# rogermm14/eonerf_code

Hardware: AMD Instinct MI355X
Metric: train rays/sec on JAX_068 (4096 rays x 128 samples) (higher is better)
Workload: dtype bf16

## Files before the change

eonerf_code_amd/csrc/eonerf_enc_pair.hip:

```cpp
#include "eonerf_common.h"
#include "eonerf_kernels.h"

namespace {

constexpr int NT = 512;
constexpr int IMG = 16 * 1024;
constexpr int ENC_B = ENC_SLOTS * SEG_B;
constexpr int SLOT_B = 2 * IMG + ENC_B;
constexpr int NS = 4, DEPTH = NS - 1;
constexpr int N_DMA = 9;
constexpr int GP_F = 4 * 32 * 4;
constexpr int SMEM_B = NS * SLOT_B + 2 * GP_F * (int)sizeof(float);

EO_DEV int swz16(int row, int chunk) { return (chunk ^ ((row >> 2) & 3)) * 16; }

EO_DEV void enc_waves(const EncPairArgs& a, uint8_t* smem, int lane, int wave, int t0, int t1, int n_pts) {
    typedef PBf16 P;
    typedef P::U U;
    const int h = lane >> 5, c = lane & 31;
    const int s_src = wave >> 1, mt = wave & 1;
    U wt[16];
#pragma unroll
    for (int kg = 0; kg < 16; ++kg) wt[kg] = *reinterpret_cast<const U*>(a.wt + ((size_t)((s_src * 2 + mt) * 16 + kg)) * 1024 + lane * 16);
    float* gp_lds = reinterpret_cast<float*>(smem + NS * SLOT_B);
    const float eoff = h ? EO_PI_2_F : 0.0f;
    auto load_pos = [&](int t, float& x, float& y, float& z) {
        const int p = t * 32 + c;
        const bool live = p < n_pts;
        x = live ? a.px[p] : 0.f; y = live ? a.py[p] : 0.f; z = live ? a.pz[p] : 0.f;
    };
    auto finish = [&](int t_prev, int par) {
        const int p = t_prev * 32 + c;
        if (h == 0 && p < n_pts) {
            const f32x4* g = reinterpret_cast<const f32x4*>(gp_lds + par * GP_F);
            f32x4 v = g[c];
#pragma unroll
            for (int w = 1; w < 4; ++w) { const f32x4 u = g[w * 32 + c]; v[0] += u[0]; v[1] += u[1]; v[2] += u[2]; }
            a.g_pos[p] = v[0]; a.g_pos[(size_t)a.p_pad + p] = v[1]; a.g_pos[2 * (size_t)a.p_pad + p] = v[2];
        }
    };
    float x, y, z;
    load_pos(t0, x, y, z);
    for (int t = t0; t < t1; ++t) {
        const int slot = (t - t0) & (NS - 1), par = (t - t0) & 1;
        asm volatile("s_barrier" ::: "memory");
        if (wave == 0 && t > t0) finish(t - 1, par ^ 1);
        const uint8_t* bp = smem + slot * SLOT_B + s_src * IMG + lane * 16;
        f32x16 acc = zero_acc();
        U fr[3];
#pragma unroll
        for (int d = 0; d < 3; ++d) fr[d] = lds_unit<P>(bp + d * 1024);
#pragma unroll
        for (int kg = 0; kg < 16; ++kg) {
            acc = P::mma(wt[kg], fr[kg % 3], acc);
            if (kg + 3 < 16) fr[kg % 3] = lds_unit<P>(bp + (kg + 3) * 1024);
        }
        float gp[3] = {0.f, 0.f, 0.f};
#pragma unroll
        for (int r = 0; r < 16; ++r) {
            const float g = acc[r];
            if (mt == 0 || r < 14) {
                const int q0 = r, q1 = 16 + r;
                const int k = mt ? q1 / 3 : q0 / 3, d = mt ? q1 % 3 : q0 % 3;
                const float cc = d == 0 ? x : (d == 1 ? y : z);
                const float arg = cc * (float)(1 << k) + eoff;
                gp[d] += g * (__cosf(arg) * (float)(1 << k));
            } else if (r == 14) {
                if (h) gp[2] += g; else gp[0] += g;
            } else {
                if (!h) gp[1] += g;
            }
        }
#pragma unroll
        for (int d = 0; d < 3; ++d) gp[d] += __shfl_xor(gp[d], 32, 64);
        if (h == 0) reinterpret_cast<f32x4*>(gp_lds + par * GP_F)[wave * 32 + c] = f32x4{gp[0], gp[1], gp[2], 0.f};
        if (t + 1 < t1) load_pos(t + 1, x, y, z);
    }
    asm volatile("s_barrier" ::: "memory");
    if (wave == 0) finish(t1 - 1, (t1 - 1 - t0) & 1);
}

EO_DEV void dw_waves(const EncPairArgs& a, uint8_t* smem, int lane, int wave, int t0, int t1) {
    typedef PBf16 P;
    typedef P::U U;
    const int h = lane >> 5, c = lane & 31, v = wave - 4;
    const int s_src = v >> 1, mhalf = v & 1;
    const size_t nt = (size_t)a.p_pad / 32;
    const uint8_t* grd = reinterpret_cast<const uint8_t*>(a.grd);
    const __amdgpu_buffer_rsrc_t rs_y0 = __builtin_amdgcn_make_buffer_rsrc(const_cast<uint8_t*>(grd) + (size_t)GRD_ROW_Y0 * nt * SEG_B, 0, -1, 0x00020000);
    const __amdgpu_buffer_rsrc_t rs_y5 = __builtin_amdgcn_make_buffer_rsrc(const_cast<uint8_t*>(grd) + (size_t)(GRD_ROW_Y0 + 5 * 256) * nt * SEG_B, 0, -1, 0x00020000);
    const __amdgpu_buffer_rsrc_t rs_e = __builtin_amdgcn_make_buffer_rsrc(const_cast<uint8_t*>(reinterpret_cast<const uint8_t*>(a.act)) + (size_t)ACT_ROW_ENC * nt * SEG_B, 0, -1, 0x00020000);
    const int enc_row = 16 * v + (lane >> 2);
    const int enc_voff = enc_row * SEG_B + (((lane & 3) ^ ((enc_row >> 2) & 3)) * 16);
    auto issue = [&](int t, int slot) {
        uint8_t* base = smem + slot * SLOT_B;
        const uint32_t so = (uint32_t)t * IMG;
#pragma unroll
        for (int i = 0; i < 4; ++i) {
            __builtin_amdgcn_raw_ptr_buffer_load_lds(rs_y0, (__attribute__((address_space(3))) void*)(base + (4 * v + i) * 1024), 16, lane * 16 + (4 * v + i) * 1024, so, 0, 2);
            __builtin_amdgcn_raw_ptr_buffer_load_lds(rs_y5, (__attribute__((address_space(3))) void*)(base + IMG + (4 * v + i) * 1024), 16, lane * 16 + (4 * v + i) * 1024, so, 0, 2);
        }
        __builtin_amdgcn_raw_ptr_buffer_load_lds(rs_e, (__attribute__((address_space(3))) void*)(base + 2 * IMG + 16 * v * SEG_B), 16, enc_voff, (uint32_t)t * ENC_B, 0, 2);
    };
    f32x16 dw[4][2];
    float dbv[4] = {0.f, 0.f, 0.f, 0.f};
#pragma unroll
    for (int i = 0; i < 4; ++i) { dw[i][0] = zero_acc(); dw[i][1] = zero_acc(); }
    const int g4 = lane >> 4, qq = (lane & 15) >> 2, pp = lane & 3;
    int off_a[4];
#pragma unroll
    for (int i = 0; i < 4; ++i)
        off_a[i] = s_src * IMG + (2 * (4 * mhalf + i) + (g4 & 1)) * 1024 + ((pp & 1) * 32 + 8 * (g4 >> 1) + qq) * 16 + (pp >> 1) * 8;
    int off_b[2][2];
#pragma unroll
    for (int j = 0; j < 2; ++j)
#pragma unroll
        for (int ks = 0; ks < 2; ++ks) { const int row = 32 * j + c; off_b[j][ks] = 2 * IMG + row * SEG_B + swz16(row, 2 * ks + h); }

#pragma unroll
    for (int d = 0; d < DEPTH; ++d) issue(t0 + d < t1 ? t0 + d : t1 - 1, d);
    for (int t = t0; t < t1; ++t) {
        const int slot = (t - t0) & (NS - 1);
        asm volatile("s_waitcnt vmcnt(%0)\n\ts_barrier" ::"n"(N_DMA * (DEPTH - 1)) : "memory");
        issue(t + DEPTH < t1 ? t + DEPTH : t1 - 1, (slot + DEPTH) & (NS - 1));
        const uint8_t* T = smem + slot * SLOT_B;
#pragma unroll
        for (int ks = 0; ks < 2; ++ks) {
            u32x2 ta[8];
            asm volatile("ds_read_b64_tr_b16 %0, %8\n\t"
                         "ds_read_b64_tr_b16 %1, %8 offset:64\n\t"
                         "ds_read_b64_tr_b16 %2, %9\n\t"
                         "ds_read_b64_tr_b16 %3, %9 offset:64\n\t"
                         "ds_read_b64_tr_b16 %4, %10\n\t"
                         "ds_read_b64_tr_b16 %5, %10 offset:64\n\t"
                         "ds_read_b64_tr_b16 %6, %11\n\t"
                         "ds_read_b64_tr_b16 %7, %11 offset:64\n\t"
                         "s_waitcnt lgkmcnt(0)"
                         : "=&v"(ta[0]), "=&v"(ta[1]), "=&v"(ta[2]), "=&v"(ta[3]), "=&v"(ta[4]), "=&v"(ta[5]), "=&v"(ta[6]), "=&v"(ta[7])
                         : "v"((uint32_t)(uintptr_t)(T + off_a[0] + 256 * ks)), "v"((uint32_t)(uintptr_t)(T + off_a[1] + 256 * ks)),
                           "v"((uint32_t)(uintptr_t)(T + off_a[2] + 256 * ks)), "v"((uint32_t)(uintptr_t)(T + off_a[3] + 256 * ks)) : "memory");
            const U b0 = lds_unit<P>(T + off_b[0][ks]), b1 = lds_unit<P>(T + off_b[1][ks]);
#pragma unroll
            for (int i = 0; i < 4; ++i) {
                const u32x4 av = u32x4{ta[2 * i][0], ta[2 * i][1], ta[2 * i + 1][0], ta[2 * i + 1][1]};
                const U af = __builtin_bit_cast(U, av);
                dw[i][0] = P::mma(af, b0, dw[i][0]);
                dw[i][1] = P::mma(af, b1, dw[i][1]);
                if (s_src == 0) {
#pragma unroll
                    for (int e = 0; e < 4; ++e) dbv[i] += __uint_as_float(av[e] << 16) + __uint_as_float(av[e] & 0xffff0000u);
                }
            }
        }
    }
    asm volatile("s_waitcnt vmcnt(0)" ::: "memory");
    float* part = a.part + (size_t)blockIdx.x * ENC_PART_F + (size_t)s_src * 256 * 64;
#pragma unroll
    for (int i = 0; i < 4; ++i)
#pragma unroll
        for (int j = 0; j < 2; ++j)
#pragma unroll
            for (int g = 0; g < 16; ++g) part[((4 * mhalf + i) * 32 + acc_row(g, h)) * 64 + 32 * j + c] = dw[i][j][g];
    if (s_src == 0) {
#pragma unroll
        for (int i = 0; i < 4; ++i) {
            const float sum = dbv[i] + __shfl_xor(dbv[i], 32, 64);
            if (h == 0) a.part[(size_t)blockIdx.x * ENC_PART_F + 2 * 256 * 64 + (4 * mhalf + i) * 32 + c] = sum;
        }
    }
}

__global__ __launch_bounds__(NT) void k_enc_pair(EncPairArgs a) {
    extern __shared__ __attribute__((aligned(16))) uint8_t smem[];
    const int lane = threadIdx.x & 63, wave = __builtin_amdgcn_readfirstlane(threadIdx.x >> 6);
    const int n_pts = *a.n_pts;
    const int n_tiles = (n_pts + 255) / 256 * 8;
    const int t0 = (int)((long long)blockIdx.x * n_tiles / gridDim.x), t1 = (int)((long long)(blockIdx.x + 1) * n_tiles / gridDim.x);
    if (t0 >= t1) {
        for (int i = threadIdx.x; i < ENC_PART_F; i += NT) a.part[(size_t)blockIdx.x * ENC_PART_F + i] = 0.f;
        return;
    }
    if (wave < 4) enc_waves(a, smem, lane, wave, t0, t1, n_pts);
    else dw_waves(a, smem, lane, wave, t0, t1);
}

}

hipError_t eo_launch_enc_pair(const EncPairArgs& a, int n_wg, hipStream_t st) {
    static EoAttrOnce attr;
    {
        const hipError_t e = attr.ensure([&] { return hipFuncSetAttribute(reinterpret_cast<const void*>(&k_enc_pair), hipFuncAttributeMaxDynamicSharedMemorySize, SMEM_B); });
        if (e != hipSuccess) return e;
    }
    hipLaunchKernelGGL(k_enc_pair, dim3(n_wg), dim3(NT), SMEM_B, st, a);
    return hipGetLastError();
}
```

Baseline: 1.244 million.

## Interleave encoding cosines with MMAs and spread DMA issue across dw compute

The encoder waves are templated on the M-tile so the cosine/frequency factors are compile-time indexed and computed between MFMA steps, with sched barriers enforcing the interleave. Position loads become buffer loads with bounds-checked descriptors and are prefetched two tiles ahead. The final gradient write is now spread across all four waves using masked buffer stores. In the dW waves, the per-tile DMA issue is split into pieces placed between MFMAs, LDS reads for both k-steps are issued up front, and fine-grained lgkmcnt waits replace the full drain. The aim is to hide the cosine latency and the LDS/DMA latency behind matrix work, at the cost of more registers and more fragile hand-written wait counts.

Result: no change. 1.250 million, median of 6 (+0.5%).

```diff
diff --git a/eonerf_code_amd/csrc/eonerf_enc_pair.hip b/eonerf_code_amd/csrc/eonerf_enc_pair.hip
--- a/eonerf_code_amd/csrc/eonerf_enc_pair.hip
+++ b/eonerf_code_amd/csrc/eonerf_enc_pair.hip
@@ -14,57 +14,75 @@
 
 EO_DEV int swz16(int row, int chunk) { return (chunk ^ ((row >> 2) & 3)) * 16; }
 
-EO_DEV void enc_waves(const EncPairArgs& a, uint8_t* smem, int lane, int wave, int t0, int t1, int n_pts) {
+template <int MT> EO_DEV void enc_waves(const EncPairArgs& a, uint8_t* smem, int lane, int wave, int t0, int t1, int n_pts) {
     typedef PBf16 P;
     typedef P::U U;
     const int h = lane >> 5, c = lane & 31;
-    const int s_src = wave >> 1, mt = wave & 1;
+    const int s_src = wave >> 1;
     U wt[16];
 #pragma unroll
-    for (int kg = 0; kg < 16; ++kg) wt[kg] = *reinterpret_cast<const U*>(a.wt + ((size_t)((s_src * 2 + mt) * 16 + kg)) * 1024 + lane * 16);
+    for (int kg = 0; kg < 16; ++kg) wt[kg] = *reinterpret_cast<const U*>(a.wt + ((size_t)((s_src * 2 + MT) * 16 + kg)) * 1024 + lane * 16);
     float* gp_lds = reinterpret_cast<float*>(smem + NS * SLOT_B);
     const float eoff = h ? EO_PI_2_F : 0.0f;
+    const uint32_t pos_b = (uint32_t)n_pts * 4u;
+    const __amdgpu_buffer_rsrc_t rs_x = __builtin_amdgcn_make_buffer_rsrc(const_cast<float*>(a.px), 0, pos_b, 0x00020000);
+    const __amdgpu_buffer_rsrc_t rs_y = __builtin_amdgcn_make_buffer_rsrc(const_cast<float*>(a.py), 0, pos_b, 0x00020000);
+    const __amdgpu_buffer_rsrc_t rs_z = __builtin_amdgcn_make_buffer_rsrc(const_cast<float*>(a.pz), 0, pos_b, 0x00020000);
+    const __amdgpu_buffer_rsrc_t rs_g = __builtin_amdgcn_make_buffer_rsrc(a.g_pos, 0, 3u * (uint32_t)a.p_pad * 4u, 0x00020000);
+    constexpr uint32_t DROP = 0x80000000u;
     auto load_pos = [&](int t, float& x, float& y, float& z) {
-        const int p = t * 32 + c;
-        const bool live = p < n_pts;
-        x = live ? a.px[p] : 0.f; y = live ? a.py[p] : 0.f; z = live ? a.pz[p] : 0.f;
-    };
-    auto finish = [&](int t_prev, int par) {
+        const uint32_t vo = (uint32_t)(t * 32 + c) * 4u;
+        x = __uint_as_float(__builtin_amdgcn_raw_buffer_load_b32(rs_x, vo, 0, 0));
+        y = __uint_as_float(__builtin_amdgcn_raw_buffer_load_b32(rs_y, vo, 0, 0));
+        z = __uint_as_float(__builtin_amdgcn_raw_buffer_load_b32(rs_z, vo, 0, 0));
+    };
+    auto finish = [&](int t_prev, int par, bool on) {
         const int p = t_prev * 32 + c;
-        if (h == 0 && p < n_pts) {
-            const f32x4* g = reinterpret_cast<const f32x4*>(gp_lds + par * GP_F);
-            f32x4 v = g[c];
-#pragma unroll
-            for (int w = 1; w < 4; ++w) { const f32x4 u = g[w * 32 + c]; v[0] += u[0]; v[1] += u[1]; v[2] += u[2]; }
-            a.g_pos[p] = v[0]; a.g_pos[(size_t)a.p_pad + p] = v[1]; a.g_pos[2 * (size_t)a.p_pad + p] = v[2];
-        }
-    };
-    float x, y, z;
-    load_pos(t0, x, y, z);
-    for (int t = t0; t < t1; ++t) {
-        const int slot = (t - t0) & (NS - 1), par = (t - t0) & 1;
+        const f32x4* g = reinterpret_cast<const f32x4*>(gp_lds + par * GP_F);
+        f32x4 v = g[c];
+#pragma unroll
+        for (int w = 1; w < 4; ++w) { const f32x4 u = g[w * 32 + c]; v[0] += u[0]; v[1] += u[1]; v[2] += u[2]; }
+        const bool mine = on && h == 0 && (c >> 3) == wave && p < n_pts;
+        const uint32_t vo = mine ? (uint32_t)p * 4u : DROP;
+        const uint32_t row = (uint32_t)a.p_pad * 4u;
+        __builtin_amdgcn_raw_buffer_store_b32(__float_as_uint(v[0]), rs_g, vo, 0, 0);
+        __builtin_amdgcn_raw_buffer_store_b32(__float_as_uint(v[1]), rs_g, vo, row, 0);
+        __builtin_amdgcn_raw_buffer_store_b32(__float_as_uint(v[2]), rs_g, vo, 2 * row, 0);
+    };
+#pragma unroll
+    for (int kg = 0; kg < 16; ++kg) asm volatile("" ::"v"(wt[kg]));
+    auto step = [&](int t, int par, float& x, float& y, float& z) {
+        const int slot = (t - t0) & (NS - 1);
         asm volatile("s_barrier" ::: "memory");
-        if (wave == 0 && t > t0) finish(t - 1, par ^ 1);
         const uint8_t* bp = smem + slot * SLOT_B + s_src * IMG + lane * 16;
         f32x16 acc = zero_acc();
+        float cf[16];
         U fr[3];
 #pragma unroll
         for (int d = 0; d < 3; ++d) fr[d] = lds_unit<P>(bp + d * 1024);
+        __builtin_amdgcn_sched_barrier(0);
 #pragma unroll
         for (int kg = 0; kg < 16; ++kg) {
             acc = P::mma(wt[kg], fr[kg % 3], acc);
             if (kg + 3 < 16) fr[kg % 3] = lds_unit<P>(bp + (kg + 3) * 1024);
-        }
+            constexpr int Q0 = 16 * MT;
+            if (Q0 + kg < 30) {
+                const int k = (Q0 + kg) / 3, d = (Q0 + kg) % 3;
+                const float cc = d == 0 ? x : (d == 1 ? y : z);
+                const float arg = __builtin_fmaf(cc, (float)(1 << k), eoff);
+                cf[kg] = __cosf(arg) * (float)(1 << k);
+            } else {
+                cf[kg] = 0.f;
+            }
+            __builtin_amdgcn_sched_barrier(0);
+        }
+        finish(t - 1, par ^ 1, t > t0);
         float gp[3] = {0.f, 0.f, 0.f};
 #pragma unroll
         for (int r = 0; r < 16; ++r) {
             const float g = acc[r];
-            if (mt == 0 || r < 14) {
-                const int q0 = r, q1 = 16 + r;
-                const int k = mt ? q1 / 3 : q0 / 3, d = mt ? q1 % 3 : q0 % 3;
-                const float cc = d == 0 ? x : (d == 1 ? y : z);
-                const float arg = cc * (float)(1 << k) + eoff;
-                gp[d] += g * (__cosf(arg) * (float)(1 << k));
+            if (MT == 0 || r < 14) {
+                gp[(16 * MT + r) % 3] = __builtin_fmaf(g, cf[r], gp[(16 * MT + r) % 3]);
             } else if (r == 14) {
                 if (h) gp[2] += g; else gp[0] += g;
             } else {
@@ -74,10 +92,19 @@
 #pragma unroll
         for (int d = 0; d < 3; ++d) gp[d] += __shfl_xor(gp[d], 32, 64);
         if (h == 0) reinterpret_cast<f32x4*>(gp_lds + par * GP_F)[wave * 32 + c] = f32x4{gp[0], gp[1], gp[2], 0.f};
-        if (t + 1 < t1) load_pos(t + 1, x, y, z);
+        load_pos(t + 2 < t1 ? t + 2 : t1 - 1, x, y, z);
+    };
+    float xa, ya, za, xb, yb, zb;
+    load_pos(t0, xa, ya, za);
+    finish(t0, 0, false);
+    load_pos(t0 + 1 < t1 ? t0 + 1 : t0, xb, yb, zb);
+    for (int t = t0; t < t1; t += 2) {
+        step(t, 0, xa, ya, za);
+        if (t + 1 >= t1) break;
+        step(t + 1, 1, xb, yb, zb);
     }
     asm volatile("s_barrier" ::: "memory");
-    if (wave == 0) finish(t1 - 1, (t1 - 1 - t0) & 1);
+    finish(t1 - 1, (t1 - 1 - t0) & 1, true);
 }
 
 EO_DEV void dw_waves(const EncPairArgs& a, uint8_t* smem, int lane, int wave, int t0, int t1) {
@@ -92,15 +119,13 @@
     const __amdgpu_buffer_rsrc_t rs_e = __builtin_amdgcn_make_buffer_rsrc(const_cast<uint8_t*>(reinterpret_cast<const uint8_t*>(a.act)) + (size_t)ACT_ROW_ENC * nt * SEG_B, 0, -1, 0x00020000);
     const int enc_row = 16 * v + (lane >> 2);
     const int enc_voff = enc_row * SEG_B + (((lane & 3) ^ ((enc_row >> 2) & 3)) * 16);
-    auto issue = [&](int t, int slot) {
+    auto issue_piece = [&](int t, int slot, int n) {
         uint8_t* base = smem + slot * SLOT_B;
         const uint32_t so = (uint32_t)t * IMG;
-#pragma unroll
-        for (int i = 0; i < 4; ++i) {
-            __builtin_amdgcn_raw_ptr_buffer_load_lds(rs_y0, (__attribute__((address_space(3))) void*)(base + (4 * v + i) * 1024), 16, lane * 16 + (4 * v + i) * 1024, so, 0, 2);
-            __builtin_amdgcn_raw_ptr_buffer_load_lds(rs_y5, (__attribute__((address_space(3))) void*)(base + IMG + (4 * v + i) * 1024), 16, lane * 16 + (4 * v + i) * 1024, so, 0, 2);
-        }
-        __builtin_amdgcn_raw_ptr_buffer_load_lds(rs_e, (__attribute__((address_space(3))) void*)(base + 2 * IMG + 16 * v * SEG_B), 16, enc_voff, (uint32_t)t * ENC_B, 0, 2);
+        const int u = 4 * v + (n >> 1);
+        if (n == 8) __builtin_amdgcn_raw_ptr_buffer_load_lds(rs_e, (__attribute__((address_space(3))) void*)(base + 2 * IMG + 16 * v * SEG_B), 16, enc_voff, (uint32_t)t * ENC_B, 0, 2);
+        else if (n & 1) __builtin_amdgcn_raw_ptr_buffer_load_lds(rs_y5, (__attribute__((address_space(3))) void*)(base + IMG + u * 1024), 16, lane * 16 + u * 1024, so, 0, 2);
+        else __builtin_amdgcn_raw_ptr_buffer_load_lds(rs_y0, (__attribute__((address_space(3))) void*)(base + u * 1024), 16, lane * 16 + u * 1024, so, 0, 2);
     };
     f32x16 dw[4][2];
     float dbv[4] = {0.f, 0.f, 0.f, 0.f};
@@ -118,34 +143,46 @@
         for (int ks = 0; ks < 2; ++ks) { const int row = 32 * j + c; off_b[j][ks] = 2 * IMG + row * SEG_B + swz16(row, 2 * ks + h); }
 
 #pragma unroll
-    for (int d = 0; d < DEPTH; ++d) issue(t0 + d < t1 ? t0 + d : t1 - 1, d);
+    for (int d = 0; d < DEPTH; ++d)
+#pragma unroll
+        for (int n = 0; n < N_DMA; ++n) issue_piece(t0 + d < t1 ? t0 + d : t1 - 1, d, n);
     for (int t = t0; t < t1; ++t) {
         const int slot = (t - t0) & (NS - 1);
         asm volatile("s_waitcnt vmcnt(%0)\n\ts_barrier" ::"n"(N_DMA * (DEPTH - 1)) : "memory");
-        issue(t + DEPTH < t1 ? t + DEPTH : t1 - 1, (slot + DEPTH) & (NS - 1));
+        const int tn = t + DEPTH < t1 ? t + DEPTH : t1 - 1, sn = (slot + DEPTH) & (NS - 1);
         const uint8_t* T = smem + slot * SLOT_B;
+        u32x2 ta[2][8];
+        u32x4 tb[2][2];
+#pragma unroll
+        for (int ks = 0; ks < 2; ++ks)
+            asm volatile("ds_read_b128 %8, %14\n\t"
+                         "ds_read_b128 %9, %15\n\t"
+                         "ds_read_b64_tr_b16 %0, %10\n\t"
+                         "ds_read_b64_tr_b16 %1, %10 offset:64\n\t"
+                         "ds_read_b64_tr_b16 %2, %11\n\t"
+                         "ds_read_b64_tr_b16 %3, %11 offset:64\n\t"
+                         "ds_read_b64_tr_b16 %4, %12\n\t"
+                         "ds_read_b64_tr_b16 %5, %12 offset:64\n\t"
+                         "ds_read_b64_tr_b16 %6, %13\n\t"
+                         "ds_read_b64_tr_b16 %7, %13 offset:64"
+                         : "=&v"(ta[ks][0]), "=&v"(ta[ks][1]), "=&v"(ta[ks][2]), "=&v"(ta[ks][3]), "=&v"(ta[ks][4]), "=&v"(ta[ks][5]), "=&v"(ta[ks][6]),
+                           "=&v"(ta[ks][7]), "=&v"(tb[ks][0]), "=&v"(tb[ks][1])
+                         : "v"((uint32_t)(uintptr_t)(T + off_a[0] + 256 * ks)), "v"((uint32_t)(uintptr_t)(T + off_a[1] + 256 * ks)),
+                           "v"((uint32_t)(uintptr_t)(T + off_a[2] + 256 * ks)), "v"((uint32_t)(uintptr_t)(T + off_a[3] + 256 * ks)),
+                           "v"((uint32_t)(uintptr_t)(T + off_b[0][ks])), "v"((uint32_t)(uintptr_t)(T + off_b[1][ks])) : "memory");
 #pragma unroll
         for (int ks = 0; ks < 2; ++ks) {
-            u32x2 ta[8];
-            asm volatile("ds_read_b64_tr_b16 %0, %8\n\t"
-                         "ds_read_b64_tr_b16 %1, %8 offset:64\n\t"
-                         "ds_read_b64_tr_b16 %2, %9\n\t"
-                         "ds_read_b64_tr_b16 %3, %9 offset:64\n\t"
-                         "ds_read_b64_tr_b16 %4, %10\n\t"
-                         "ds_read_b64_tr_b16 %5, %10 offset:64\n\t"
-                         "ds_read_b64_tr_b16 %6, %11\n\t"
-                         "ds_read_b64_tr_b16 %7, %11 offset:64\n\t"
-                         "s_waitcnt lgkmcnt(0)"
-                         : "=&v"(ta[0]), "=&v"(ta[1]), "=&v"(ta[2]), "=&v"(ta[3]), "=&v"(ta[4]), "=&v"(ta[5]), "=&v"(ta[6]), "=&v"(ta[7])
-                         : "v"((uint32_t)(uintptr_t)(T + off_a[0] + 256 * ks)), "v"((uint32_t)(uintptr_t)(T + off_a[1] + 256 * ks)),
-                           "v"((uint32_t)(uintptr_t)(T + off_a[2] + 256 * ks)), "v"((uint32_t)(uintptr_t)(T + off_a[3] + 256 * ks)) : "memory");
-            const U b0 = lds_unit<P>(T + off_b[0][ks]), b1 = lds_unit<P>(T + off_b[1][ks]);
 #pragma unroll
             for (int i = 0; i < 4; ++i) {
-                const u32x4 av = u32x4{ta[2 * i][0], ta[2 * i][1], ta[2 * i + 1][0], ta[2 * i + 1][1]};
+                constexpr int LEFT[2][4] = {{15, 14, 12, 10}, {6, 4, 2, 0}};
+                if (i == 0) asm volatile("s_waitcnt lgkmcnt(%4)" : "+v"(ta[ks][0]), "+v"(ta[ks][1]), "+v"(tb[ks][0]), "+v"(tb[ks][1]) : "n"(LEFT[ks][0]));
+                else asm volatile("s_waitcnt lgkmcnt(%2)" : "+v"(ta[ks][2 * i]), "+v"(ta[ks][2 * i + 1]) : "n"(LEFT[ks][i]));
+                const u32x4 av = u32x4{ta[ks][2 * i][0], ta[ks][2 * i][1], ta[ks][2 * i + 1][0], ta[ks][2 * i + 1][1]};
                 const U af = __builtin_bit_cast(U, av);
-                dw[i][0] = P::mma(af, b0, dw[i][0]);
-                dw[i][1] = P::mma(af, b1, dw[i][1]);
+                dw[i][0] = P::mma(af, __builtin_bit_cast(U, tb[ks][0]), dw[i][0]);
+                dw[i][1] = P::mma(af, __builtin_bit_cast(U, tb[ks][1]), dw[i][1]);
+                if (ks == 0 && i == 0) issue_piece(tn, sn, 8);
+                issue_piece(tn, sn, 4 * ks + i);
                 if (s_src == 0) {
 #pragma unroll
                     for (int e = 0; e < 4; ++e) dbv[i] += __uint_as_float(av[e] << 16) + __uint_as_float(av[e] & 0xffff0000u);
@@ -180,8 +217,9 @@
         for (int i = threadIdx.x; i < ENC_PART_F; i += NT) a.part[(size_t)blockIdx.x * ENC_PART_F + i] = 0.f;
         return;
     }
-    if (wave < 4) enc_waves(a, smem, lane, wave, t0, t1, n_pts);
-    else dw_waves(a, smem, lane, wave, t0, t1);
+    if (wave >= 4) dw_waves(a, smem, lane, wave, t0, t1);
+    else if (wave & 1) enc_waves<1>(a, smem, lane, wave, t0, t1, n_pts);
+    else enc_waves<0>(a, smem, lane, wave, t0, t1, n_pts);
 }
 
 }
```
